# xiph/daala

Measured on AMD Instinct MI355X. Metric: 1080p all-intra transform blocks/s (filter+DCT+PVQ), higher is better.
Workload: dtype int32 (lifting DCT/filters) + f64 (PVQ search)

## Files before the change

### daala_amd/csrc/pvq_refbands.hip

```cpp
#include "../../include/daala_hip.h"
#include <math.h>
#include <stdio.h>
#include <stdlib.h>
#include <string.h>
#include "od_ctx.cuh"
#include "od_pvq_math.cuh"
#include "od_occupancy.cuh"
#include "od_krange.cuh"
#include "od_band_stage.cuh"
#include "gen/od_scan_tables.h"
#define OD_RSQ_TABLE_N 512
#define OD_RSQ_HUGE
#include "pvq_search.cuh"
#include "pvq_row.cuh"
#include "pvq_regs.cuh"
#include "pvq_lane.cuh"

namespace {

constexpr int kMaxJobs = 8;
constexpr int kMaxItems = kMaxJobs*ODHIP_MAX_BANDS;
constexpr int kSlots = ODHIP_PVQ_REF_SLOTS;
constexpr int kUncCap = 1 << 16;
constexpr double kDefaultMargin = 1e-9;
// ... 59 lines not shown
    const int yv = (int16_t)(yw[e >> 1] >> (16*(e & 1)));
    const int qmi = (int16_t)(qw[e >> 1] >> (16*(e & 1)));
    rv[e] = odq_shr_round(odq_mult16_32_q16(yv, ch.z)*qmi, ch.w);
  }
}

__device__ __forceinline__ void lref_piece(const RJob &jb, int band, long blk, int c0, int (&rv)[8]) {
  const long lblk = lref_block(jb, blk);
  const int4 ch = reinterpret_cast<const int4 *>(jb.lchoice)[lblk*jb.lnb + band];
  uint4 y4 = make_uint4(0, 0, 0, 0);
  if (ch.y != 0) y4 = *reinterpret_cast<const uint4 *>(jb.ly + ((long)ch.x*jb.lnblocks + lblk)*jb.llen + c0);
  lref_dequant(ch, y4, *reinterpret_cast<const uint4 *>(jb.lqmi + c0), rv);
}

struct Unc;
struct PUncR {
  int job;
  int band;
  unsigned blk;
  int reserved;
  double rate[ODHIP_PVQ_REF_SLOTS + 1];
};
constexpr int kPUncCap = 1 << 14;

struct RItems : ItemTable<kMaxItems> {
  int perturb;
  double lambda;
  double margin;
  const RJob *jobs;
  unsigned *unc_count;
  Unc *unc;
  unsigned *pcount;
  struct PUncR *plist;
  double tol_scale;
  int fuse;
  int sort_weights;
#ifdef ODHIP_EXPERIMENTS
  int abl;
#endif
};

struct Unc {
  int job;
  int band;
  unsigned blk;
  int theta;
  double corr;
};

__constant__ unsigned char kRScanXY[OD_SCAN_LEN][2];

__device__ __forceinline__ long block_base(const RJob &j, long blk) {
  const int N = 4 << j.bs;
  const long per = (long)j.bw*j.bh;
  const int p = (int)(blk/per);
// ... 61 lines not shown
  const int proj_shift = (odq_ilog(abs(proj)) - 1) - 14;
  const int16_t proj_norm = (int16_t)odq_vshr_round(proj, proj_shift);
  *proj_1 = (int16_t)odq_mult16_16_q15(proj_norm, rcp);
  int os = 14 - proj_shift - 1 + l2r_shift;
  *outshift = os > 30 ? 30 : os;
}


constexpr int kSortBins = 256;
constexpr int kSortChunk = 2048;

__device__ __forceinline__ int od_work_bin(int pulses) {
  if (pulses < 96) return pulses;
  const int b = 96 + ((pulses - 96) >> 3);
  return b < kSortBins ? b : kSortBins - 1;
}

template <class Sink>
__device__ __forceinline__ void refb_enumerate(const RJob &jb, int band, int32_t cg, int32_t gain_offset,
 int32_t theta, int flags, double corr, Sink &sink) {
  const int n = jb.off[band + 1] - jb.off[band];
  const int beta = jb.beta[band];
  if (flags & ODHIP_REFBAND_THETA) {
    int nth = 0;
    const int gain_bound = (cg - gain_offset) >> ODQ_CGAIN_SHIFT;
    const double scale_1 = __ddiv_rn(1., kThetaScale);
    for (int i = gain_bound - 1 > 1 ? gain_bound - 1 : 1; i <= gain_bound + 1; i++) {
      const int32_t qcg = odq_shl32(i, ODQ_CGAIN_SHIFT) + gain_offset;
      const int ts = odq_pvq_compute_max_theta(qcg, beta);
      const double t = __ddiv_rn(((theta*scale_1)*2), kPi)*ts;
      int lower = (int)floor(.5 + t) - 2;
      if (lower < 0) lower = 0;
      int upper = (int)ceil(t);
      if (upper > ts - 1) upper = ts - 1;
      const int gi = i - (gain_bound - 1);
      sink.gain(gi, i, ts, lower);
      for (int j = lower; j <= upper && nth < ODHIP_PVQ_REF_SLOTS - 2; j++) {
        sink.theta(gi, i, j, ts, odq_compute_k_ref(j, n));
        nth++;
      }
    }
  }
  if ((jb.is_keyframe && jb.pli == 0) || corr < .5 || cg < odq_shl32(2, ODQ_CGAIN_SHIFT)) {
    const int gain_bound = cg >> ODQ_CGAIN_SHIFT;
    int c = 0;
    for (int i = gain_bound > 1 ? gain_bound : 1; i <= gain_bound + 1; i++) {
      sink.noref(c++, i, odq_compute_k_noref(odq_shl32(i, ODQ_CGAIN_SHIFT), n, beta));
    }
  }
}

struct KeySink {
  int kt = 0;
  int kn = 0;
  int c = 0;
  unsigned long long mt = 0;
  unsigned long long mn = 0;
  __device__ __forceinline__ void gain(int, int, int, int) {}
// ... 23 lines not shown
    if (fabs(u - rint(u)) < it.margin) {
      flags |= ODHIP_REFBAND_UNCERTAIN;
      if (it.perturb & 1) theta += 1;
      const unsigned slot = atomicAdd(it.unc_count, 1u);
      if (slot < (unsigned)kUncCap) {
        Unc e;
        e.job = job;
        e.band = band;
        e.blk = (unsigned)blk;
        e.theta = theta;
        e.corr = p.corr;
        it.unc[slot] = e;
      }
    }
  }
  odhip_pvq_refband o;
  o.xshift = xshift;
  o.rshift = rshift;
  o.g = p.g;
  o.gr = p.gr;
  o.cg = p.cg;
  o.cgr = p.cgr;
  o.icgr = p.icgr;
  o.gain_offset = p.gain_offset;
  o.m = (int16_t)m;
  o.s = (int8_t)s;
  o.flags = (uint8_t)flags;
  o.theta = theta;
  o.nitems = 0;
  o.ntheta = 0;
  o.corr = p.corr;
  o.dist0 = p.dist0;
  *rec = o;
  if (it.fuse == 2) {
    KeySink ks;
    refb_enumerate(jb, band, o.cg, o.gain_offset, o.theta, flags, o.corr, ks);
    jb.keys[(long)band*jb.nblocks + blk] = (unsigned short)(kSortBins - 1 - od_work_bin(ks.work(it.sort_weights)));
    if (ks.kt > ODHIP_PVQ_MAX_K || ks.kn > ODHIP_PVQ_MAX_K) atomicAdd(jb.krange, 1u);
  }
}

__device__ __forceinline__ uint32_t pack16(int lo, int hi) {
  return (uint32_t)(lo & 0xffff) | (uint32_t)hi << 16;
}

template <int E, class YGet>
__device__ __forceinline__ void store_pulses(int16_t *dst, YGet y) {
  constexpr int SH = E == 15 ? 1 : 0;
  static_assert((E + SH) % 8 == 0, "whole 16-byte pieces");
  uint4 *p = reinterpret_cast<uint4 *>(dst - SH);
  int t[E + SH];
  if (SH) t[0] = 0;
#pragma unroll
  for (int i = 0; i < E; i++) t[i + SH] = y(i);
// ... 191 lines not shown
    for (int i = 0; i < N; i++) {
      int32_t tmp = odq_mult16_16(r16[i], proj_1);
      tmp = outshift >= 0 ? odq_shr_round(tmp, outshift) : odq_shl32(tmp, -outshift);
      v[i] = (int16_t)(x16[i] - tmp);
    }
#pragma unroll
    for (int i = 0; i < N - 1; i++) xr[i] = i < m ? v[i] : v[i + 1];
  }
#ifdef ODHIP_EXPERIMENTS
  const bool abl_nostore = (it.abl & 1) != 0;
  const bool abl_norec = (it.abl & 4) != 0;
#else
  constexpr bool abl_nostore = false;
  constexpr bool abl_norec = false;
#endif
  if (abl_nostore) {
  }
  else if (N == 15) {
    uint4 *xo = reinterpret_cast<uint4 *>(x16o);
    uint4 *ro = reinterpret_cast<uint4 *>(r16o);
    uint4 *xro4 = reinterpret_cast<uint4 *>(xro);
    xo[0] = make_uint4(pack16(0, x16[0]), pack16(x16[1], x16[2]), pack16(x16[3], x16[4]),
     pack16(x16[5], x16[6]));
    xo[1] = make_uint4(pack16(x16[7], x16[8]), pack16(x16[9], x16[10]), pack16(x16[11], x16[12]),
     pack16(x16[13], x16[N - 1]));
    ro[0] = make_uint4(pack16(0, r16[0]), pack16(r16[1], r16[2]), pack16(r16[3], r16[4]),
     pack16(r16[5], r16[6]));
    ro[1] = make_uint4(pack16(r16[7], r16[8]), pack16(r16[9], r16[10]), pack16(r16[11], r16[12]),
     pack16(r16[13], r16[N - 1]));
    xro4[0] = make_uint4(pack16(0, xr[0]), pack16(xr[1], xr[2]), pack16(xr[3], xr[4]),
     pack16(xr[5], xr[6]));
    xro4[1] = make_uint4(pack16(xr[7], xr[8]), pack16(xr[9], xr[10]), pack16(xr[11], xr[12]),
     pack16(xr[13], 0));
  }
  else {
    *reinterpret_cast<uint4 *>(x16o + off) = make_uint4(pack16(x16[0], x16[1]), pack16(x16[2], x16[3]),
     pack16(x16[4], x16[5]), pack16(x16[6], x16[7]));
    *reinterpret_cast<uint4 *>(r16o + off) = make_uint4(pack16(r16[0], r16[1]), pack16(r16[2], r16[3]),
     pack16(r16[4], r16[5]), pack16(r16[6], r16[7]));
    *reinterpret_cast<uint4 *>(xro + off) = make_uint4(pack16(xr[0], xr[1]), pack16(xr[2], xr[3]),
     pack16(xr[4], xr[5]), pack16(xr[6], 0));
  }
  if (!abl_norec) {
    prep_write(it, jb, jb.rec + blk*jb.nb_bands + band, job, band, blk, xshift, rshift, p, r_null, flip, m, s);
  }
}

__global__ __launch_bounds__(kWave) void k_refb_prep_corner(RItems it) {
  const int item = find_item(it, blockIdx.x);
  const int job = __builtin_amdgcn_readfirstlane(it.job[item]);
  const RJob jb = it.jobs[job];
  const long blk = (long)(blockIdx.x - it.wg_start[item])*kWave + threadIdx.x;
  if (blk >= jb.nblocks) return;
  const bool more = jb.nb_bands > 1;
  const int w = jb.w;
  const long base = block_base(jb, blk);
// ... 128 lines not shown
      lref_piece(jb, band, blk, 0, lo);
      lref_piece(jb, band, blk, 8, hi);
#pragma unroll
      for (int i = 0; i < N; i++) rv[i] = i + 1 < 8 ? lo[(i + 1) & 7] : hi[(i + 1) & 7];
    }
    else {
      int pc[8];
      lref_piece(jb, band, blk, off, pc);
#pragma unroll
      for (int i = 0; i < N; i++) rv[i] = pc[i & 7];
    }
  }
  int flip = 0;
  if (jb.is_keyframe && jb.pli != 0) {
    if constexpr (N == 15) flip = cfl_flip15(xv, rv, const_table(jb.qm + off));
    else flip = (jb.rec[blk*jb.nb_bands].flags & ODHIP_REFBAND_FLIP) != 0;
  }
  prep_lane_band<N>(it, jb, job, band, blk, off, xv, rv, flip);
}
#endif

template <int E, int G>
__global__ __launch_bounds__(kWave) void k_refb_prep_row(RItems it) {
  constexpr int n = G*E;
  __shared__ unsigned short s_scan[n];
  const int item = find_item(it, blockIdx.x);
  const int job = it.job[item];
  const RJob &jb = it.jobs[job];
  const int band = it.band[item];
  const int off = jb.off[band];
  const int lane = threadIdx.x;
  for (int j = lane; j < n; j += kWave) s_scan[j] = gRScanPk[off + j];
  __syncthreads();
  const int row = lane/G;
  const int l = lane%G;
  const long nblocks = jb.nblocks;
  const long blk0 = (long)(blockIdx.x - it.wg_start[item])*(kWave/G) + row;
  const bool live = blk0 < nblocks;
  const long blk = live ? blk0 : nblocks - 1;
  const int w = jb.w;
  const int len = jb.len;
  const int nb_bands = jb.nb_bands;
  const int q0 = job_q(jb, band, blk);
  const int beta = jb.beta[band];
  const int is_keyframe = jb.is_keyframe;
  const int cfl_enabled = is_keyframe && jb.pli != 0;
  const long base = block_base(jb, blk);
  const od_coeff *x0 = jb.coef + base;
  const bool lref = jb.ly != nullptr;
  const od_coeff *r0 = lref ? jb.coef + base : jb.ref + base;
  const int16_t *qmp = jb.qm + off + l*E;
  odhip_pvq_refband *rec = jb.rec + blk*nb_bands;
  int16_t *x16o = jb.x16 + blk*len + off;
  int16_t *r16o = jb.r16 + blk*len + off;
  int16_t *xro = jb.xr + blk*len + off;
  const int flip = cfl_enabled ? (rec[0].flags & ODHIP_REFBAND_FLIP) != 0 : 0;
  int xv[E];
  int rv[E];
  int qm[E];
  int sx = 0;
  int sr = 0;
  int nz = 0;
#pragma unroll
  for (int e = 0; e < E; e++) {
    const int pk = s_scan[l*E + e];
    const long p = (long)(pk >> 8)*w + (pk & 255);
    xv[e] = x0[p];
    const int r = lref ? 0 : r0[p];
    rv[e] = flip ? -r : r;
    qm[e] = qmp[e];
  }
// ... 82 lines not shown
    l2r = grp_sum<G>(l2r);
    proj = grp_sum<G>(proj);
    int16_t proj_1;
    int outshift;
    householder_consts(l2r, proj, &proj_1, &outshift);
#pragma unroll
    for (int e = 0; e < E; e++) {
      const int i = l*E + e;
      int32_t tmp = odq_mult16_16(r16[e], proj_1);
      tmp = outshift >= 0 ? odq_shr_round(tmp, outshift) : odq_shl32(tmp, -outshift);
      const int16_t v = (int16_t)(x16[e] - tmp);
      if (live && i != m) xro[i - (i > m)] = v;
    }
  }
  if (live) {
    if constexpr (E == 8) {
      *reinterpret_cast<uint4 *>(x16o + l*E) = make_uint4(pack16(x16[0], x16[1]),
       pack16(x16[2], x16[3]), pack16(x16[4], x16[5]), pack16(x16[6], x16[7]));
      *reinterpret_cast<uint4 *>(r16o + l*E) = make_uint4(pack16(r16[0], r16[1]),
       pack16(r16[2], r16[3]), pack16(r16[4], r16[5]), pack16(r16[6], r16[7]));
    }
    else {
#pragma unroll
      for (int e = 0; e < E; e += 2) {
        *reinterpret_cast<uint32_t *>(x16o + l*E + e) = pack16(x16[e], x16[e + 1]);
        *reinterpret_cast<uint32_t *>(r16o + l*E + e) = pack16(r16[e], r16[e + 1]);
      }
    }
    if (l == 0) prep_write(it, jb, rec + band, job, band, blk, xshift, rshift, p, r_null, flip, m, s);
  }
}


struct ItemPtr {
  int4 *head;
  int4 *tail;
  int4 *res;
  long stride;
};

__device__ __forceinline__ ItemPtr item_ptr(const RJob &jb, int band, long blk) {
  ItemPtr p;
  const long plane = (long)jb.nb_bands*kSlots*jb.nblocks;
  p.head = reinterpret_cast<int4 *>(jb.items) + (long)band*kSlots*jb.nblocks + blk;
// ... 548 lines not shown
  return l == 0 ? 0 : t;
}

template <int G>
__device__ __forceinline__ int grp_total(int v) {
  if constexpr (G == 1) return v;
  else if constexpr (G == 2) return od_grp_add<2>(v);
  else return grp_sum<G>(v);
}

struct RefOutcome {
  int qg;
  int skip;
};

__device__ __forceinline__ RefOutcome refb_decide(const RItems &it, int job, const RJob &jb, int band, long blk,
 const odhip_pvq_refband &r, const RefBest &best, bool writer, int4 *ch) {
  const int cfl_enabled = jb.is_keyframe && jb.pli != 0;
  const int noref = best.noref;
  RefOutcome o;
  o.qg = 0;
  int itheta = jb.is_keyframe ? -1 : 0;
  int max_theta = 0;
  int best_k = 0;
  if (best.close && writer) {
    const unsigned slot = atomicAdd(it.pcount, 1u);
    if (slot < (unsigned)kPUncCap) {
      PUncR *e = it.plist + slot;
      e->job = job;
      e->band = band;
      e->blk = (unsigned)blk;
    }
// ... 20 lines not shown
    if (qg == r.icgr && itheta == 0 && !cfl_enabled) o.skip = 2;
  }
  if (writer) {
    ch[0] = make_int4(best.chosen, qg, noref, itheta);
    ch[1] = make_int4(max_theta, best_k, o.skip, jb.is_keyframe ? (noref ? qg : neg_interleave(qg, r.icgr))
     : (noref ? qg - 1 : neg_interleave(qg + 1, r.icgr + 1)));
  }
  if (o.skip && writer) {
    const int flip = (r.flags & ODHIP_REFBAND_FLIP) != 0;
    ch[2] = make_int4(o.skip == 2 ? (flip ? 4 : 1) : 0, -1, 0, 0);
    ch[3] = make_int4(0, 0, 0, 0);
  }
  return o;
}

template <int E, int G, bool STORE, class YGet>
__device__ __forceinline__ void refb_finish(const RItems &it, int job, const RJob &jb, int band, long blk,
 const odhip_pvq_refband &r, const RefBest &best, int l, bool live, YGet y) {
  constexpr int SH = E == 15 ? 1 : 0;
  static_assert(G == 1 || SH == 0, "only a whole band in one lane starts inside a 16-byte piece");
  const bool writer = live && l == 0;
  int4 *ch = reinterpret_cast<int4 *>(jb.choice + (blk*jb.nb_bands + band)*16);
  const RefOutcome o = refb_decide(it, job, jb, band, blk, r, best, writer, ch);
  if (o.skip) return;
  const int noref = best.noref;
  const int yslot = best.yslot;
  const long at = blk*jb.len + jb.off[band] + l*E;
  int wy[E];
#pragma unroll
  for (int e = 0; e < E; e++) wy[e] = y(e);
  if (STORE && live && yslot >= 0) store_pulses<E>(jb.y + at, [&](int e) -> int { return wy[e]; });
  const int32_t g = odq_gain_expand(odq_shl32(o.qg, ODQ_CGAIN_SHIFT) + (noref ? 0 : r.gain_offset),
   job_q(jb, band, blk), jb.beta[band]);
// ... 9 lines not shown
  gshift = gshift > 0 ? gshift : 0;
  int32_t scale = 0;
  if (yy != 0) {
    int rsqrt_shift;
    const int16_t rsqrt = odq_rsqrt(yy, &rsqrt_shift);
    scale = odq_vshr_round(rsqrt*(int64_t)g, rsqrt_shift + gshift - 16);
  }
  const int qshift = ODQ_QM_INV_SHIFT - gshift;
  if (noref) {
    if (writer) {
      ch[2] = make_int4(2, yslot, scale, qshift);
      ch[3] = make_int4(0, 0, 0, 0);
    }
    return;
  }
  const odhip_pvq_refband *rec = jb.rec + (blk*jb.nb_bands + band);
  const int m = rec->m;
  const int s = rec->s;
  scale = (int32_t)floor(.5 + (scale*(1./32768))*odq_pvq_sin(best.qtheta));
  const int16_t xm = (int16_t)floor(.5 + ((-s*odq_shr_round(g, gshift))*(1./32768))*odq_pvq_cos(best.qtheta));
  uint32_t rw[(E + SH)/2];
  {
    const uint4 *rp = reinterpret_cast<const uint4 *>(jb.r16 + at - SH);
#pragma unroll
    for (int q = 0; q < (E + SH)/8; q++) {
      const uint4 r4 = rp[q];
      rw[4*q] = r4.x;
      rw[4*q + 1] = r4.y;
      rw[4*q + 2] = r4.z;
      rw[4*q + 3] = r4.w;
    }
  }
  const int yprev = grp_from_prev<G>(wy[E - 1], l);
// ... 269 lines not shown
    while (pos > 0) {
      const uint32_t q = col[(pos - 1)*stride];
      if ((q & 0x3ffffu) <= (c & 0x3ffffu)) break;
      if (writer) col[pos*stride] = q;
      pos--;
    }
    if (writer) col[pos*stride] = c;
    n++;
  }
  __device__ __forceinline__ void noref(int c, int, int k) {
    if (writer) col[n*stride] = (uint32_t)c | (uint32_t)(k < 65535 ? k : 65535) << 2;
    n++;
  }
};

__device__ __forceinline__ CandList refb_build_list(const RJob &jb, int band, const odhip_pvq_refband &r,
 uint32_t *col, int stride, bool writer) {
  ListSink sink;
  sink.col = col;
  sink.stride = stride;
  sink.writer = writer;
  CandList cl;
  cl.col = col;
  cl.stride = stride;
  cl.gb1 = ((r.cg - r.gain_offset) >> ODQ_CGAIN_SHIFT) - 1;
  const int gbn = r.cg >> ODQ_CGAIN_SHIFT;
  cl.gbn = gbn > 1 ? gbn : 1;
  struct Split {
    ListSink &s;
    int ntheta = -1;
    __device__ __forceinline__ void gain(int gi, int i, int ts, int lower) { s.gain(gi, i, ts, lower); }
// ... 20 lines not shown
  ThetaCand c;
  c.gi = (int)(w & 3u);
  c.i = cl.gb1 + c.gi;
  c.ts = (int)cl.col[(kSlots + c.gi)*cl.stride];
  c.j = (int)cl.col[(kSlots + 3 + c.gi)*cl.stride] + (int)(w >> 18);
  return c;
}

struct ThetaGate {
  int32_t qcg;
  int32_t qtheta;
  int cosd;
  bool skip;
};

__device__ __forceinline__ ThetaGate refb_theta_gate(const odhip_pvq_refband &r, const ThetaCand &c, int k,
 double lambda) {
  ThetaGate g;
  g.qcg = odq_shl32(c.i, ODQ_CGAIN_SHIFT) + r.gain_offset;
  g.qtheta = odq_pvq_compute_theta(c.j, c.ts);
  g.cosd = odq_pvq_cos(r.theta - g.qtheta);
  g.skip = (refb_dist_gate(g.qcg, r.cg, refb_cos_term(g.cosd)) > r.dist0 + 1.0*lambda && k != 0)
   || k > ODHIP_PVQ_MAX_K;
  return g;
}

struct PreInline {
  ThetaGate g;
  __device__ __forceinline__ void prepare(const odhip_pvq_refband &, const CandList &, double) {}
  __device__ __forceinline__ bool skip(const odhip_pvq_refband &r, const ThetaCand &c, int, int k, double lambda) {
    g = refb_theta_gate(r, c, k, lambda);
    return g.skip;
  }
  __device__ __forceinline__ void values(const odhip_pvq_refband &r, const ThetaCand &, int, int32_t &qcg,
   double &sin_prod) const {
    qcg = g.qcg;
    sin_prod = refb_sin_prod(odq_pvq_sin(r.theta), odq_pvq_sin(g.qtheta));
  }
  __device__ __forceinline__ double cos_term(const odhip_pvq_refband &r, int) const {
    return refb_cos_term(odq_pvq_cos(r.theta - g.qtheta));
  }
};

template <int G, class Store>
__device__ __forceinline__ void refb_prepass(const odhip_pvq_refband &r, const CandList &cl, double lambda, int l,
 Store store) {
  for (int c = l; c < kSlots; c += G) {
    if (c < cl.ntheta) {
      const uint32_t w = cl.col[c*cl.stride];
      store(c, refb_theta_gate(r, theta_cand(cl, w), (int)(w >> 2 & 0xffffu), lambda));
    }
  }
}

template <int WAVES>
__device__ __forceinline__ void refb_prepass_fence(void) {
  if constexpr (WAVES == 1) __syncthreads();
  else {
    __builtin_amdgcn_fence(__ATOMIC_RELEASE, "wavefront");
    __builtin_amdgcn_wave_barrier();
    __builtin_amdgcn_fence(__ATOMIC_ACQUIRE, "wavefront");
  }
}

constexpr int kPreWords = 6;
template <int G, int WAVES>
struct PreLds {
  uint32_t *pre;
  int stride;
  int l;
  double cos = 0;
  __device__ __forceinline__ void prepare(const odhip_pvq_refband &r, const CandList &cl, double lambda) {
    refb_prepass<G>(r, cl, lambda, l, [&](int c, const ThetaGate &g) {
      const double cos_term = refb_cos_term(g.cosd);
      const double sin_prod = refb_sin_prod(odq_pvq_sin(r.theta), odq_pvq_sin(g.qtheta));
      uint32_t *p = pre + c*kPreWords*stride;
      p[0] = (uint32_t)g.qcg;
      p[stride] = g.skip;
      p[2*stride] = (uint32_t)__double2loint(cos_term);
      p[3*stride] = (uint32_t)__double2hiint(cos_term);
      p[4*stride] = (uint32_t)__double2loint(sin_prod);
      p[5*stride] = (uint32_t)__double2hiint(sin_prod);
    });
    refb_prepass_fence<WAVES>();
  }
  __device__ __forceinline__ bool skip(const odhip_pvq_refband &, const ThetaCand &, int idx, int, double) const {
    return pre[(idx*kPreWords + 1)*stride] != 0;
  }
  __device__ __forceinline__ void values(const odhip_pvq_refband &, const ThetaCand &, int idx, int32_t &qcg,
   double &sin_prod) {
    const uint32_t *p = pre + idx*kPreWords*stride;
    qcg = (int32_t)p[0];
    cos = __hiloint2double((int)p[3*stride], (int)p[2*stride]);
    sin_prod = __hiloint2double((int)p[5*stride], (int)p[4*stride]);
  }
  __device__ __forceinline__ double cos_term(const odhip_pvq_refband &, int) const { return cos; }
};

constexpr int kPrePacked = 1;
template <int G, int WAVES>
struct PrePacked {
  static_assert((G == 2 || G == 4) && kSlots <= 32, "the parts of a group's skip mask");
  uint32_t *pre;
  int stride;
  int l;
  uint32_t skips = 0;
  double cos = 0;
  __device__ __forceinline__ void prepare(const odhip_pvq_refband &r, const CandList &cl, double lambda) {
    refb_prepass<G>(r, cl, lambda, l, [&](int c, const ThetaGate &g) {
      skips |= (uint32_t)g.skip << c;
      pre[c*kPrePacked*stride] = ((uint32_t)g.cosd & 0xffffu) | (uint32_t)odq_pvq_sin(g.qtheta) << 16;
    });
    skips = od_grp_or<G>(skips);
    refb_prepass_fence<WAVES>();
  }
  __device__ __forceinline__ bool skip(const odhip_pvq_refband &, const ThetaCand &, int idx, int, double) const {
    return (skips >> idx & 1u) != 0;
  }
  __device__ __forceinline__ void values(const odhip_pvq_refband &r, const ThetaCand &c, int idx, int32_t &qcg,
   double &sin_prod) {
    const uint32_t cs = pre[idx*kPrePacked*stride];
    qcg = odq_shl32(c.i, ODQ_CGAIN_SHIFT) + r.gain_offset;
    cos = refb_cos_term((int16_t)(cs & 0xffffu));
    sin_prod = refb_sin_prod(odq_pvq_sin(r.theta), (int16_t)(cs >> 16));
  }
  __device__ __forceinline__ double cos_term(const odhip_pvq_refband &, int) const { return cos; }
};

template <class D>
__device__ __forceinline__ int lean_k(const D &dec, uint32_t w) {
#ifdef ODHIP_EXPERIMENTS
  if (dec.abl & 8) return 0;
#endif
  (void)dec;
  return (int)(w >> 2 & 0xffffu);
}

template <int NR, class Pre, class V, class D>
__device__ __forceinline__ void refb_loops_lean(const RJob &jb, int band, long blk, const odhip_pvq_refband &r,
 const CandList &cl, double lambda, V &v, D &dec, Pre &pre) {
  const int off = jb.off[band];
  const int n = jb.off[band + 1] - off;
  const int len = jb.len;
  const int32_t cg = r.cg;
  pre.prepare(r, cl, lambda);
  if (cl.ntheta > 0) {
    v.load(jb.xr + blk*len + off, true);
    int prev_k = 0;
    bool has = false;
    double cos_dist = 0;
    double prate = 0;
    int idx = 0;
    while (idx < cl.ntheta) {
      const uint32_t w = cl.col[idx*cl.stride];
// ... 50 lines not shown
template <int NY>
struct LeanDecide {
  double best_cost;
  int chosen;
  bool close;
  int y[NY];
  typename LeanSigns<NY>::type sg;
  double lambda;
  double tol_scale;
  int icgr;
  int is_keyframe;
  int pli;
#ifdef ODHIP_EXPERIMENTS
  int abl = 0;
#endif
  __device__ __forceinline__ void init(const odhip_pvq_refband &r, const RJob &jb, double lam, double tol) {
    best_cost = r.dist0;
    chosen = -1;
    close = false;
    lambda = lam;
    tol_scale = tol;
    icgr = r.icgr;
    is_keyframe = jb.is_keyframe;
    pli = jb.pli;
    sg = 0;
#pragma unroll
    for (int i = 0; i < NY; i++) y[i] = 0;
  }
  template <class V>
  __device__ __forceinline__ void offer(int idx, bool with_ref, int i, int j, double dist, double prate,
   double lts, bool has, const V &v) {
// ... 44 lines not shown
  }
  return b;
}

template <int E, int G>
struct LeanBand {
  int wave;
  int lane;
  int row;
  int l;
  int job;
  int band;
  const RJob *jb;
  bool live;
  long blk;
  odhip_pvq_refband r;
  CandList cl;
  LeanDecide<E> dec;
};

template <int E, int G, int WAVES>
__device__ __forceinline__ bool lean_band(const RItems &it, uint32_t (&s_list_w)[WAVES][kLeanWords*(kWave/G)],
 LeanBand<E, G> &b) {
  constexpr int C = kWave/G;
  b.wave = __builtin_amdgcn_readfirstlane(threadIdx.x/kWave);
  const int unit = blockIdx.x*WAVES + b.wave;
  if (unit >= it.wg_start[it.nitems]) return false;
  const int item = find_item(it, unit);
  b.job = it.job[item];
  b.jb = &it.jobs[b.job];
  b.band = it.band[item];
  b.lane = threadIdx.x%kWave;
  b.row = b.lane/G;
  b.l = b.lane%G;
  const RJob &jb = *b.jb;
  const long nblocks = jb.nblocks;
  const long pos = (long)(unit - it.wg_start[item])*C + b.row;
  b.live = pos < nblocks;
  if (G == 1 && !b.live) return false;
  b.blk = jb.ids[(long)b.band*nblocks + (b.live ? pos : nblocks - 1)];
  b.r = jb.rec[b.blk*jb.nb_bands + b.band];
  b.cl = refb_build_list(jb, b.band, b.r, s_list_w[b.wave] + b.row, C, b.l == 0);
  b.dec.init(b.r, jb, it.lambda, it.tol_scale);
#ifdef ODHIP_EXPERIMENTS
  b.dec.abl = it.abl;
#endif
  return true;
}

template <int N>
__global__ __launch_bounds__(kSearchThreads) OD_SEARCH_OCC_ATTR void k_refb_lean_lane(RItems it) {
  __shared__ uint32_t s_list_w[kSearchWaves][kLeanWords*kWave];
  OD_SEARCH_VGPR_FLOOR();
  od_rsqrt_init(threadIdx.x);
  LeanBand<N, 1> b;
  if (!lean_band<N, 1, kSearchWaves>(it, s_list_w, b)) return;
// ... 294 lines not shown
    d.lqmi = l.d_qm_inv;
    d.lsplit = (long)l.nplanes*d.bw*d.bh;
    d.lnblocks = d.lsplit;
    d.llen = ln*ln < OD_SCAN_LEN ? ln*ln : OD_SCAN_LEN;
    d.lnb = OD_NBANDS[l.bs];
  }
  return ODHIP_SUCCESS;
}

struct RefState {
  long theta_listed = 0;
  JobTables<RJob, kMaxJobs> tabs;
  Counters<3> counters;
  DeviceBuf<Unc> unc;
  DeviceBuf<PUncR> plist;
  PinnedCount unc_posted;
  PinnedCount priced;
  BlockSort<kSortBins, kSortChunk, RJob, kMaxItems> sort;
  SideStreams streams;
  ProfEvents prof;
  double margin = kDefaultMargin;
  int perturb = 0;
  double tol_scale = 1.;
  bool lean = false;
  unsigned *unc_count() const { return counters.d.p; }
  unsigned *pcount() const { return counters.d.p + 1; }
};

int ref_state(RefState **out) {
  ODHIP_CTX_OR_RETURN(ctx);
// ... 42 lines not shown
  return w;
}

void items_begin(RItems &it, const RefState &st, double lambda) {
  memset(&it, 0, sizeof(it));
  it.lambda = lambda;
  it.margin = st.margin;
  it.perturb = st.perturb;
  it.jobs = st.tabs.cur;
  it.unc_count = st.unc_count();
  it.unc = st.unc.p;
  it.pcount = st.pcount();
  it.plist = st.plist.p;
  it.tol_scale = st.tol_scale;
  it.sort_weights = sort_weights();
#ifdef ODHIP_EXPERIMENTS
  static const int abl = [] {
    const char *e = getenv("ODHIP_REFB_ABL");
    return e ? atoi(e) : 0;
  }();
  it.abl = abl;
#endif
}

enum RefStage {
  kStageRecords = 0,
  kStageLanePriced = 1,
  kStageDecided = 2
};

// ... 118 lines not shown
    }
#endif
  }
  if (st.streams.join(s, side) != ODHIP_SUCCESS) return ODHIP_EFAULT;
  return ODHIP_SUCCESS;
}

int ref_bands(const odhip_pvq_refjob *jobs, int njobs, double pvq_norm_lambda, odhip_stream stream, RefStage stage) {
  hipStream_t s = (hipStream_t)stream;
  REF_STATE_OR_RETURN(st);
  RJob host[kMaxJobs];
  int rc = stage_jobs(st, jobs, njobs, kJobBands, host, s);
  if (rc) return rc;
  ODHIP_TRY(hipMemsetAsync(st.unc_count(), 0, (stage != kStageRecords ? 2 : 1)*sizeof(unsigned), s));
  st.lean = stage == kStageDecided;
  RItems it;
  items_begin(it, st, pvq_norm_lambda);
  items_add_size(it, host, njobs, 0, kWave);
  if (!it.nitems) return ODHIP_SUCCESS;
  launch_prep(st, host, njobs, pvq_norm_lambda, stage, s);
  if (stage != kStageDecided) k_refb_cands<<<it.wg_start[it.nitems], kWave, 0, s>>>(it);
  rc = sort_blocks(st, host, njobs, s);
  if (rc) return rc;
  rc = launch_searches(st, host, njobs, pvq_norm_lambda, stage, s);
  if (rc) return rc;
  if (stage == kStageDecided) {
    rc = st.unc_posted.post(st.unc_count(), s);
    if (!rc) rc = st.priced.post(st.pcount(), s);
    if (rc) return rc;
  }
  return odhip_check_launch();
}

void rerun_listed(const RefState &st, const Unc *d_list, unsigned n, double lambda, hipStream_t s) {
  k_refb_cands_list<<<(n + kWave - 1)/kWave, kWave, 0, s>>>(st.tabs.cur, d_list, (int)n);
  k_refb_search_list<<<n, kWave, (size_t)2*128*kWave*sizeof(unsigned short), s>>>(st.tabs.cur, d_list, (int)n,
   lambda);
}

void decide_listed(RefState &st, const Unc *d_list, unsigned n, double lambda, hipStream_t s) {
  RItems it;
  items_begin(it, st, lambda);
  const unsigned grid = (n + kWave - 1)/kWave;
  for (const int size : kBandSizes) {
    for_band_size(size, [&](auto N) {
      k_refb_choose_unc_list<decltype(N)::value><<<grid, kWave, 0, s>>>(it, d_list, (int)n);
    });
  }
  (void)st.priced.post(st.pcount(), s);
}

enum RefSelect {
// ... 114 lines not shown
  for (int i = 0; i < count; i++) {
    const int32_t theta = (int32_t)floor(.5 + (32768*2./M_PI)*acos(list[i].corr));
    if (theta != list[i].theta) {
      list[nfix] = list[i];
      list[nfix].theta = theta;
      nfix++;
    }
  }
  if (nfix == 0) return 0;
  RJob host[kMaxJobs];
  int rc = stage_jobs(st, jobs, njobs, kJobBands, host, s);
  if (rc) return rc;
  if (!listed_jobs_valid(list.data(), nfix, njobs)) return ODHIP_EINVAL;
  DeviceBuf<Unc> d_list;
  if (upload_list(d_list, list.data(), nfix, &s)) return ODHIP_EFAULT;
  rerun_listed(st, d_list.p, nfix, pvq_norm_lambda, s);
  if (st.lean) decide_listed(st, d_list.p, nfix, pvq_norm_lambda, s);
  rc = odhip_check_launch();
  const hipError_t e = hipStreamSynchronize(s);
  if (rc) return rc;
  if (e != hipSuccess) return ODHIP_EFAULT;
  return (int)nfix;
}

int odhip_pvq_ref_resolve_finish(const odhip_pvq_refjob *jobs, int njobs, double pvq_norm_lambda,
 odhip_stream stream) {
  REF_STATE_OR_RETURN(st);
  const int posted = st.unc_posted.wait();
  if (posted <= 0) return posted;
  return odhip_pvq_ref_resolve(jobs, njobs, pvq_norm_lambda, stream);
// ... 41 lines not shown
    catch (const std::bad_alloc &) {
      return ODHIP_EFAULT;
    }
    for (int i = 0; i < count; i++) {
      ul[i].job = list[i].job;
      ul[i].band = list[i].band;
      ul[i].blk = list[i].blk;
      ul[i].theta = -1;
      ul[i].corr = 0;
    }
    DeviceBuf<Unc> d_ul;
    if (upload_list(d_ul, ul.data(), count)) return ODHIP_EFAULT;
    RJob host0[kMaxJobs];
    rc = stage_jobs(st, jobs, njobs, kJobBands, host0, s);
    if (rc) return rc;
    rerun_listed(st, d_ul.p, count, pvq_norm_lambda, s);
    rc = odhip_check_launch();
    if (hipStreamSynchronize(s) != hipSuccess) rc = ODHIP_EFAULT;
    if (!rc) rc = stage_jobs(st, jobs, njobs, kJobChoice, host, s);
    if (rc) return rc;
  }
  for (PUncR &e : list) {
    const RJob &jb = host[e.job];
    const int n = jb.off[e.band + 1] - jb.off[e.band];
    const long B = jb.nblocks;
    odhip_pvq_refband rec;
    ODHIP_TRY(hipMemcpy(&rec, jb.rec + (long)e.blk*jb.nb_bands + e.band, sizeof(rec), hipMemcpyDeviceToHost));
    const int4 *head = reinterpret_cast<const int4 *>(jb.items) + (long)e.band*kSlots*B + e.blk;
    const int4 *tail = head + (long)jb.nb_bands*kSlots*B;
    for (int c = 0; c <= kSlots; c++) e.rate[c] = 0;
// ... 46 lines not shown
```

Before: 1.317 billion.

## Write compact lean per-band records and skip unused x/xr stores in fused mode

In the fused (lean) decide path, the prep kernels now write a compact 32-byte LeanRec per band into a separate buffer instead of the full odhip_pvq_refband record. They also skip storing x16 when no no-ref candidates exist and xr when no Householder reflection was applied. The lean decide kernels read the compact record and unpack the derived values. The uncertain-list rerun paths gain a new prep_list kernel that rebuilds full records for listed bands. This cuts global write and read traffic in the common path, at the cost of an extra buffer, more code paths, and an added kernel launch on the resolve paths.

```diff
diff --git a/daala_amd/csrc/pvq_refbands.hip b/daala_amd/csrc/pvq_refbands.hip
--- a/daala_amd/csrc/pvq_refbands.hip
+++ b/daala_amd/csrc/pvq_refbands.hip
@@ -97,6 +97,42 @@
 }
 
 struct Unc;
+struct LeanRec {
+  int32_t cg;
+  int32_t cgr;
+  int32_t theta;
+  uint32_t msf;
+  double corr;
+  double dist0;
+};
+static_assert(sizeof(LeanRec) == 32, "two records to a 64-byte line");
+
+struct LeanVals {
+  int32_t cg;
+  int32_t gain_offset;
+  int32_t icgr;
+  int32_t theta;
+  int flags;
+  double corr;
+  double dist0;
+};
+
+__device__ __forceinline__ uint32_t lean_msf(int m, int s, int flags) {
+  return (uint32_t)(uint16_t)m | (uint32_t)(uint8_t)s << 16 | (uint32_t)flags << 24;
+}
+
+__device__ __forceinline__ LeanVals lean_vals(const LeanRec &m) {
+  LeanVals r;
+  r.cg = m.cg;
+  r.icgr = odq_shr_round(m.cgr, ODQ_CGAIN_SHIFT);
+  r.gain_offset = m.cgr - odq_shl32(r.icgr, ODQ_CGAIN_SHIFT);
+  r.theta = m.theta;
+  r.flags = (int)(m.msf >> 24);
+  r.corr = m.corr;
+  r.dist0 = m.dist0;
+  return r;
+}
+
 struct PUncR {
   int job;
   int band;
@@ -121,7 +157,18 @@
 #ifdef ODHIP_EXPERIMENTS
   int abl;
 #endif
+  LeanRec *lean;
+  long lean_at[kMaxJobs];
 };
+
+__device__ __forceinline__ LeanRec *lean_rec(const RItems &it, int job, const RJob &jb, long blk, int band) {
+  return it.lean + (it.lean_at[job] + blk*jb.nb_bands + band);
+}
+
+__device__ __forceinline__ int block_flip(const RItems &it, int job, const RJob &jb, long blk, bool lean) {
+  const int flags = lean ? (int)(lean_rec(it, job, jb, blk, 0)->msf >> 24) : jb.rec[blk*jb.nb_bands].flags;
+  return (flags & ODHIP_REFBAND_FLIP) != 0;
+}
 
 struct Unc {
   int job;
@@ -213,6 +260,10 @@
   if (pulses < 96) return pulses;
   const int b = 96 + ((pulses - 96) >> 3);
   return b < kSortBins ? b : kSortBins - 1;
+}
+
+__device__ __forceinline__ bool refb_has_noref(const RJob &jb, int32_t cg, double corr) {
+  return (jb.is_keyframe && jb.pli == 0) || corr < .5 || cg < odq_shl32(2, ODQ_CGAIN_SHIFT);
 }
 
 template <class Sink>
@@ -240,7 +291,7 @@
       }
     }
   }
-  if ((jb.is_keyframe && jb.pli == 0) || corr < .5 || cg < odq_shl32(2, ODQ_CGAIN_SHIFT)) {
+  if (refb_has_noref(jb, cg, corr)) {
     const int gain_bound = cg >> ODQ_CGAIN_SHIFT;
     int c = 0;
     for (int i = gain_bound > 1 ? gain_bound : 1; i <= gain_bound + 1; i++) {
@@ -294,6 +345,21 @@
       }
     }
   }
+  if (it.fuse == 2) {
+    LeanRec o;
+    o.cg = p.cg;
+    o.cgr = p.cgr;
+    o.theta = theta;
+    o.msf = lean_msf(m, s, flags);
+    o.corr = p.corr;
+    o.dist0 = p.dist0;
+    *lean_rec(it, job, jb, blk, band) = o;
+    KeySink ks;
+    refb_enumerate(jb, band, p.cg, p.gain_offset, theta, flags, p.corr, ks);
+    jb.keys[(long)band*jb.nblocks + blk] = (unsigned short)(kSortBins - 1 - od_work_bin(ks.work(it.sort_weights)));
+    if (ks.kt > ODHIP_PVQ_MAX_K || ks.kn > ODHIP_PVQ_MAX_K) atomicAdd(jb.krange, 1u);
+    return;
+  }
   odhip_pvq_refband o;
   o.xshift = xshift;
   o.rshift = rshift;
@@ -312,12 +378,6 @@
   o.corr = p.corr;
   o.dist0 = p.dist0;
   *rec = o;
-  if (it.fuse == 2) {
-    KeySink ks;
-    refb_enumerate(jb, band, o.cg, o.gain_offset, o.theta, flags, o.corr, ks);
-    jb.keys[(long)band*jb.nblocks + blk] = (unsigned short)(kSortBins - 1 - od_work_bin(ks.work(it.sort_weights)));
-    if (ks.kt > ODHIP_PVQ_MAX_K || ks.kn > ODHIP_PVQ_MAX_K) atomicAdd(jb.krange, 1u);
-  }
 }
 
 __device__ __forceinline__ uint32_t pack16(int lo, int hi) {
@@ -539,32 +599,42 @@
   constexpr bool abl_nostore = false;
   constexpr bool abl_norec = false;
 #endif
+  const bool keep_x = it.fuse != 2 || refb_has_noref(jb, p.cg, p.corr);
+  const bool keep_xr = it.fuse != 2 || p.ran;
   if (abl_nostore) {
   }
   else if (N == 15) {
     uint4 *xo = reinterpret_cast<uint4 *>(x16o);
     uint4 *ro = reinterpret_cast<uint4 *>(r16o);
     uint4 *xro4 = reinterpret_cast<uint4 *>(xro);
-    xo[0] = make_uint4(pack16(0, x16[0]), pack16(x16[1], x16[2]), pack16(x16[3], x16[4]),
-     pack16(x16[5], x16[6]));
-    xo[1] = make_uint4(pack16(x16[7], x16[8]), pack16(x16[9], x16[10]), pack16(x16[11], x16[12]),
-     pack16(x16[13], x16[N - 1]));
+    if (keep_x) {
+      xo[0] = make_uint4(pack16(0, x16[0]), pack16(x16[1], x16[2]), pack16(x16[3], x16[4]),
+       pack16(x16[5], x16[6]));
+      xo[1] = make_uint4(pack16(x16[7], x16[8]), pack16(x16[9], x16[10]), pack16(x16[11], x16[12]),
+       pack16(x16[13], x16[N - 1]));
+    }
     ro[0] = make_uint4(pack16(0, r16[0]), pack16(r16[1], r16[2]), pack16(r16[3], r16[4]),
      pack16(r16[5], r16[6]));
     ro[1] = make_uint4(pack16(r16[7], r16[8]), pack16(r16[9], r16[10]), pack16(r16[11], r16[12]),
      pack16(r16[13], r16[N - 1]));
-    xro4[0] = make_uint4(pack16(0, xr[0]), pack16(xr[1], xr[2]), pack16(xr[3], xr[4]),
-     pack16(xr[5], xr[6]));
-    xro4[1] = make_uint4(pack16(xr[7], xr[8]), pack16(xr[9], xr[10]), pack16(xr[11], xr[12]),
-     pack16(xr[13], 0));
+    if (keep_xr) {
+      xro4[0] = make_uint4(pack16(0, xr[0]), pack16(xr[1], xr[2]), pack16(xr[3], xr[4]),
+       pack16(xr[5], xr[6]));
+      xro4[1] = make_uint4(pack16(xr[7], xr[8]), pack16(xr[9], xr[10]), pack16(xr[11], xr[12]),
+       pack16(xr[13], 0));
+    }
   }
   else {
-    *reinterpret_cast<uint4 *>(x16o + off) = make_uint4(pack16(x16[0], x16[1]), pack16(x16[2], x16[3]),
-     pack16(x16[4], x16[5]), pack16(x16[6], x16[7]));
+    if (keep_x) {
+      *reinterpret_cast<uint4 *>(x16o + off) = make_uint4(pack16(x16[0], x16[1]), pack16(x16[2], x16[3]),
+       pack16(x16[4], x16[5]), pack16(x16[6], x16[7]));
+    }
     *reinterpret_cast<uint4 *>(r16o + off) = make_uint4(pack16(r16[0], r16[1]), pack16(r16[2], r16[3]),
      pack16(r16[4], r16[5]), pack16(r16[6], r16[7]));
-    *reinterpret_cast<uint4 *>(xro + off) = make_uint4(pack16(xr[0], xr[1]), pack16(xr[2], xr[3]),
-     pack16(xr[4], xr[5]), pack16(xr[6], 0));
+    if (keep_xr) {
+      *reinterpret_cast<uint4 *>(xro + off) = make_uint4(pack16(xr[0], xr[1]), pack16(xr[2], xr[3]),
+       pack16(xr[4], xr[5]), pack16(xr[6], 0));
+    }
   }
   if (!abl_norec) {
     prep_write(it, jb, jb.rec + blk*jb.nb_bands + band, job, band, blk, xshift, rshift, p, r_null, flip, m, s);
@@ -723,28 +793,19 @@
   int flip = 0;
   if (jb.is_keyframe && jb.pli != 0) {
     if constexpr (N == 15) flip = cfl_flip15(xv, rv, const_table(jb.qm + off));
-    else flip = (jb.rec[blk*jb.nb_bands].flags & ODHIP_REFBAND_FLIP) != 0;
+    else flip = block_flip(it, job, jb, blk, it.fuse == 2);
   }
   prep_lane_band<N>(it, jb, job, band, blk, off, xv, rv, flip);
 }
 #endif
 
 template <int E, int G>
-__global__ __launch_bounds__(kWave) void k_refb_prep_row(RItems it) {
+__device__ __forceinline__ void prep_row_band(const RItems &it, int job, const RJob &jb, int band, long blk0,
+ bool lean_flip, const unsigned short *s_scan) {
   constexpr int n = G*E;
-  __shared__ unsigned short s_scan[n];
-  const int item = find_item(it, blockIdx.x);
-  const int job = it.job[item];
-  const RJob &jb = it.jobs[job];
-  const int band = it.band[item];
   const int off = jb.off[band];
-  const int lane = threadIdx.x;
-  for (int j = lane; j < n; j += kWave) s_scan[j] = gRScanPk[off + j];
-  __syncthreads();
-  const int row = lane/G;
-  const int l = lane%G;
+  const int l = threadIdx.x%G;
   const long nblocks = jb.nblocks;
-  const long blk0 = (long)(blockIdx.x - it.wg_start[item])*(kWave/G) + row;
   const bool live = blk0 < nblocks;
   const long blk = live ? blk0 : nblocks - 1;
   const int w = jb.w;
@@ -763,7 +824,7 @@
   int16_t *x16o = jb.x16 + blk*len + off;
   int16_t *r16o = jb.r16 + blk*len + off;
   int16_t *xro = jb.xr + blk*len + off;
-  const int flip = cfl_enabled ? (rec[0].flags & ODHIP_REFBAND_FLIP) != 0 : 0;
+  const int flip = cfl_enabled ? block_flip(it, job, jb, blk, lean_flip) : 0;
   int xv[E];
   int rv[E];
   int qm[E];
@@ -876,20 +937,106 @@
     }
   }
   if (live) {
+    const bool keep_x = it.fuse != 2 || refb_has_noref(jb, p.cg, p.corr);
     if constexpr (E == 8) {
-      *reinterpret_cast<uint4 *>(x16o + l*E) = make_uint4(pack16(x16[0], x16[1]),
-       pack16(x16[2], x16[3]), pack16(x16[4], x16[5]), pack16(x16[6], x16[7]));
+      if (keep_x) {
+        *reinterpret_cast<uint4 *>(x16o + l*E) = make_uint4(pack16(x16[0], x16[1]),
+         pack16(x16[2], x16[3]), pack16(x16[4], x16[5]), pack16(x16[6], x16[7]));
+      }
       *reinterpret_cast<uint4 *>(r16o + l*E) = make_uint4(pack16(r16[0], r16[1]),
        pack16(r16[2], r16[3]), pack16(r16[4], r16[5]), pack16(r16[6], r16[7]));
     }
     else {
 #pragma unroll
       for (int e = 0; e < E; e += 2) {
-        *reinterpret_cast<uint32_t *>(x16o + l*E + e) = pack16(x16[e], x16[e + 1]);
+        if (keep_x) *reinterpret_cast<uint32_t *>(x16o + l*E + e) = pack16(x16[e], x16[e + 1]);
         *reinterpret_cast<uint32_t *>(r16o + l*E + e) = pack16(r16[e], r16[e + 1]);
       }
     }
     if (l == 0) prep_write(it, jb, rec + band, job, band, blk, xshift, rshift, p, r_null, flip, m, s);
+  }
+}
+
+template <int E, int G>
+__global__ __launch_bounds__(kWave) void k_refb_prep_row(RItems it) {
+  constexpr int n = G*E;
+  __shared__ unsigned short s_scan[n];
+  const int item = find_item(it, blockIdx.x);
+  const int job = it.job[item];
+  const RJob &jb = it.jobs[job];
+  const int band = it.band[item];
+  const int off = jb.off[band];
+  const int lane = threadIdx.x;
+  for (int j = lane; j < n; j += kWave) s_scan[j] = gRScanPk[off + j];
+  __syncthreads();
+  const long blk0 = (long)(blockIdx.x - it.wg_start[item])*(kWave/G) + lane/G;
+  prep_row_band<E, G>(it, job, jb, band, blk0, it.fuse == 2, s_scan);
+}
+
+template <int N>
+__device__ __forceinline__ void prep_lane_listed(const RItems &it, int job, const RJob &jb, int band, long blk) {
+  const int off = jb.off[band];
+  const long base = block_base(jb, blk);
+  const bool lref = jb.ly != nullptr;
+  int xv[N];
+  int rv[N];
+#pragma unroll
+  for (int i = 0; i < N; i++) {
+    const long p = base + coef_pos(jb, off + i);
+    xv[i] = jb.coef[p];
+    rv[i] = lref ? 0 : jb.ref[p];
+  }
+  if (lref) {
+    if constexpr (N == 15) {
+      int lo[8];
+      int hi[8];
+      lref_piece(jb, band, blk, 0, lo);
+      lref_piece(jb, band, blk, 8, hi);
+#pragma unroll
+      for (int i = 0; i < N; i++) rv[i] = i + 1 < 8 ? lo[(i + 1) & 7] : hi[(i + 1) & 7];
+    }
+    else {
+      int pc[8];
+      lref_piece(jb, band, blk, off, pc);
+#pragma unroll
+      for (int i = 0; i < N; i++) rv[i] = pc[i & 7];
+    }
+  }
+  int flip = 0;
+  if (jb.is_keyframe && jb.pli != 0) {
+    if constexpr (N == 15) flip = cfl_flip15(xv, rv, const_table(jb.qm + off));
+    else flip = block_flip(it, job, jb, blk, true);
+  }
+  prep_lane_band<N>(it, jb, job, band, blk, off, xv, rv, flip);
+}
+
+__global__ __launch_bounds__(kWave) void k_refb_prep_list(RItems it, const Unc *list, int count) {
+  __shared__ unsigned short s_scan[128];
+  if ((int)blockIdx.x >= count) return;
+  const Unc e = list[blockIdx.x];
+  const int job = e.job;
+  const RJob &jb = it.jobs[job];
+  const int band = e.band;
+  const long blk = e.blk;
+  const int off = jb.off[band];
+  const int n = jb.off[band + 1] - off;
+  const int lane = threadIdx.x;
+  if (n >= 32) {
+    for (int j = lane; j < n; j += kWave) s_scan[j] = gRScanPk[off + j];
+    __syncthreads();
+    if (n == 32) prep_row_band<8, 4>(it, job, jb, band, lane < 4 ? blk : jb.nblocks, true, s_scan);
+    else prep_row_band<8, 16>(it, job, jb, band, lane < 16 ? blk : jb.nblocks, true, s_scan);
+  }
+  else if (lane == 0) {
+    if (n == 15) prep_lane_listed<15>(it, job, jb, band, blk);
+    else prep_lane_listed<8>(it, job, jb, band, blk);
+  }
+  if (lane == 0) {
+    LeanRec *lr = lean_rec(it, job, jb, blk, band);
+    odhip_pvq_refband *rec = jb.rec + blk*jb.nb_bands + band;
+    if (e.theta >= 0) lr->theta = e.theta;
+    rec->theta = lr->theta;
+    rec->flags = (uint8_t)(lr->msf >> 24);
   }
 }
 
@@ -1468,8 +1615,9 @@
   int skip;
 };
 
+template <class R>
 __device__ __forceinline__ RefOutcome refb_decide(const RItems &it, int job, const RJob &jb, int band, long blk,
- const odhip_pvq_refband &r, const RefBest &best, bool writer, int4 *ch) {
+ const R &r, const RefBest &best, bool writer, int4 *ch) {
   const int cfl_enabled = jb.is_keyframe && jb.pli != 0;
   const int noref = best.noref;
   RefOutcome o;
@@ -1520,9 +1668,23 @@
   return o;
 }
 
-template <int E, int G, bool STORE, class YGet>
+__device__ __forceinline__ void band_pivot(const RItems &, int, const RJob &jb, int band, long blk,
+ const odhip_pvq_refband &, int &m, int &s) {
+  const odhip_pvq_refband *rec = jb.rec + (blk*jb.nb_bands + band);
+  m = rec->m;
+  s = rec->s;
+}
+
+__device__ __forceinline__ void band_pivot(const RItems &it, int job, const RJob &jb, int band, long blk,
+ const LeanVals &, int &m, int &s) {
+  const uint32_t w = lean_rec(it, job, jb, blk, band)->msf;
+  m = (int)(w & 0xffffu);
+  s = (int8_t)(w >> 16);
+}
+
+template <int E, int G, bool STORE, class R, class YGet>
 __device__ __forceinline__ void refb_finish(const RItems &it, int job, const RJob &jb, int band, long blk,
- const odhip_pvq_refband &r, const RefBest &best, int l, bool live, YGet y) {
+ const R &r, const RefBest &best, int l, bool live, YGet y) {
   constexpr int SH = E == 15 ? 1 : 0;
   static_assert(G == 1 || SH == 0, "only a whole band in one lane starts inside a 16-byte piece");
   const bool writer = live && l == 0;
@@ -1562,9 +1724,9 @@
     }
     return;
   }
-  const odhip_pvq_refband *rec = jb.rec + (blk*jb.nb_bands + band);
-  const int m = rec->m;
-  const int s = rec->s;
+  int m;
+  int s;
+  band_pivot(it, job, jb, band, blk, r, m, s);
   scale = (int32_t)floor(.5 + (scale*(1./32768))*odq_pvq_sin(best.qtheta));
   const int16_t xm = (int16_t)floor(.5 + ((-s*odq_shr_round(g, gshift))*(1./32768))*odq_pvq_cos(best.qtheta));
   uint32_t rw[(E + SH)/2];
@@ -1864,7 +2026,7 @@
   }
 };
 
-__device__ __forceinline__ CandList refb_build_list(const RJob &jb, int band, const odhip_pvq_refband &r,
+__device__ __forceinline__ CandList refb_build_list(const RJob &jb, int band, const LeanVals &r,
  uint32_t *col, int stride, bool writer) {
   ListSink sink;
   sink.col = col;
@@ -1915,7 +2077,7 @@
   bool skip;
 };
 
-__device__ __forceinline__ ThetaGate refb_theta_gate(const odhip_pvq_refband &r, const ThetaCand &c, int k,
+__device__ __forceinline__ ThetaGate refb_theta_gate(const LeanVals &r, const ThetaCand &c, int k,
  double lambda) {
   ThetaGate g;
   g.qcg = odq_shl32(c.i, ODQ_CGAIN_SHIFT) + r.gain_offset;
@@ -1928,23 +2090,23 @@
 
 struct PreInline {
   ThetaGate g;
-  __device__ __forceinline__ void prepare(const odhip_pvq_refband &, const CandList &, double) {}
-  __device__ __forceinline__ bool skip(const odhip_pvq_refband &r, const ThetaCand &c, int, int k, double lambda) {
+  __device__ __forceinline__ void prepare(const LeanVals &, const CandList &, double) {}
+  __device__ __forceinline__ bool skip(const LeanVals &r, const ThetaCand &c, int, int k, double lambda) {
     g = refb_theta_gate(r, c, k, lambda);
     return g.skip;
   }
-  __device__ __forceinline__ void values(const odhip_pvq_refband &r, const ThetaCand &, int, int32_t &qcg,
+  __device__ __forceinline__ void values(const LeanVals &r, const ThetaCand &, int, int32_t &qcg,
    double &sin_prod) const {
     qcg = g.qcg;
     sin_prod = refb_sin_prod(odq_pvq_sin(r.theta), odq_pvq_sin(g.qtheta));
   }
-  __device__ __forceinline__ double cos_term(const odhip_pvq_refband &r, int) const {
+  __device__ __forceinline__ double cos_term(const LeanVals &r, int) const {
     return refb_cos_term(odq_pvq_cos(r.theta - g.qtheta));
   }
 };
 
 template <int G, class Store>
-__device__ __forceinline__ void refb_prepass(const odhip_pvq_refband &r, const CandList &cl, double lambda, int l,
+__device__ __forceinline__ void refb_prepass(const LeanVals &r, const CandList &cl, double lambda, int l,
  Store store) {
   for (int c = l; c < kSlots; c += G) {
     if (c < cl.ntheta) {
@@ -1971,7 +2133,7 @@
   int stride;
   int l;
   double cos = 0;
-  __device__ __forceinline__ void prepare(const odhip_pvq_refband &r, const CandList &cl, double lambda) {
+  __device__ __forceinline__ void prepare(const LeanVals &r, const CandList &cl, double lambda) {
     refb_prepass<G>(r, cl, lambda, l, [&](int c, const ThetaGate &g) {
       const double cos_term = refb_cos_term(g.cosd);
       const double sin_prod = refb_sin_prod(odq_pvq_sin(r.theta), odq_pvq_sin(g.qtheta));
@@ -1985,17 +2147,17 @@
     });
     refb_prepass_fence<WAVES>();
   }
-  __device__ __forceinline__ bool skip(const odhip_pvq_refband &, const ThetaCand &, int idx, int, double) const {
+  __device__ __forceinline__ bool skip(const LeanVals &, const ThetaCand &, int idx, int, double) const {
     return pre[(idx*kPreWords + 1)*stride] != 0;
   }
-  __device__ __forceinline__ void values(const odhip_pvq_refband &, const ThetaCand &, int idx, int32_t &qcg,
+  __device__ __forceinline__ void values(const LeanVals &, const ThetaCand &, int idx, int32_t &qcg,
    double &sin_prod) {
     const uint32_t *p = pre + idx*kPreWords*stride;
     qcg = (int32_t)p[0];
     cos = __hiloint2double((int)p[3*stride], (int)p[2*stride]);
     sin_prod = __hiloint2double((int)p[5*stride], (int)p[4*stride]);
   }
-  __device__ __forceinline__ double cos_term(const odhip_pvq_refband &, int) const { return cos; }
+  __device__ __forceinline__ double cos_term(const LeanVals &, int) const { return cos; }
 };
 
 constexpr int kPrePacked = 1;
@@ -2007,7 +2169,7 @@
   int l;
   uint32_t skips = 0;
   double cos = 0;
-  __device__ __forceinline__ void prepare(const odhip_pvq_refband &r, const CandList &cl, double lambda) {
+  __device__ __forceinline__ void prepare(const LeanVals &r, const CandList &cl, double lambda) {
     refb_prepass<G>(r, cl, lambda, l, [&](int c, const ThetaGate &g) {
       skips |= (uint32_t)g.skip << c;
       pre[c*kPrePacked*stride] = ((uint32_t)g.cosd & 0xffffu) | (uint32_t)odq_pvq_sin(g.qtheta) << 16;
@@ -2015,17 +2177,17 @@
     skips = od_grp_or<G>(skips);
     refb_prepass_fence<WAVES>();
   }
-  __device__ __forceinline__ bool skip(const odhip_pvq_refband &, const ThetaCand &, int idx, int, double) const {
+  __device__ __forceinline__ bool skip(const LeanVals &, const ThetaCand &, int idx, int, double) const {
     return (skips >> idx & 1u) != 0;
   }
-  __device__ __forceinline__ void values(const odhip_pvq_refband &r, const ThetaCand &c, int idx, int32_t &qcg,
+  __device__ __forceinline__ void values(const LeanVals &r, const ThetaCand &c, int idx, int32_t &qcg,
    double &sin_prod) {
     const uint32_t cs = pre[idx*kPrePacked*stride];
     qcg = odq_shl32(c.i, ODQ_CGAIN_SHIFT) + r.gain_offset;
     cos = refb_cos_term((int16_t)(cs & 0xffffu));
     sin_prod = refb_sin_prod(odq_pvq_sin(r.theta), (int16_t)(cs >> 16));
   }
-  __device__ __forceinline__ double cos_term(const odhip_pvq_refband &, int) const { return cos; }
+  __device__ __forceinline__ double cos_term(const LeanVals &, int) const { return cos; }
 };
 
 template <class D>
@@ -2038,7 +2200,7 @@
 }
 
 template <int NR, class Pre, class V, class D>
-__device__ __forceinline__ void refb_loops_lean(const RJob &jb, int band, long blk, const odhip_pvq_refband &r,
+__device__ __forceinline__ void refb_loops_lean(const RJob &jb, int band, long blk, const LeanVals &r,
  const CandList &cl, double lambda, V &v, D &dec, Pre &pre) {
   const int off = jb.off[band];
   const int n = jb.off[band + 1] - off;
@@ -2119,7 +2281,7 @@
 #ifdef ODHIP_EXPERIMENTS
   int abl = 0;
 #endif
-  __device__ __forceinline__ void init(const odhip_pvq_refband &r, const RJob &jb, double lam, double tol) {
+  __device__ __forceinline__ void init(const LeanVals &r, const RJob &jb, double lam, double tol) {
     best_cost = r.dist0;
     chosen = -1;
     close = false;
@@ -2194,7 +2356,7 @@
   const RJob *jb;
   bool live;
   long blk;
-  odhip_pvq_refband r;
+  LeanVals r;
   CandList cl;
   LeanDecide<E> dec;
 };
@@ -2219,7 +2381,7 @@
   b.live = pos < nblocks;
   if (G == 1 && !b.live) return false;
   b.blk = jb.ids[(long)b.band*nblocks + (b.live ? pos : nblocks - 1)];
-  b.r = jb.rec[b.blk*jb.nb_bands + b.band];
+  b.r = lean_vals(*lean_rec(it, b.job, jb, b.blk, b.band));
   b.cl = refb_build_list(jb, b.band, b.r, s_list_w[b.wave] + b.row, C, b.l == 0);
   b.dec.init(b.r, jb, it.lambda, it.tol_scale);
 #ifdef ODHIP_EXPERIMENTS
@@ -2544,6 +2706,8 @@
   Counters<3> counters;
   DeviceBuf<Unc> unc;
   DeviceBuf<PUncR> plist;
+  DeviceBuf<LeanRec> lean_rec;
+  long lean_at[kMaxJobs] = {};
   PinnedCount unc_posted;
   PinnedCount priced;
   BlockSort<kSortBins, kSortChunk, RJob, kMaxItems> sort;
@@ -2616,6 +2780,8 @@
   it.plist = st.plist.p;
   it.tol_scale = st.tol_scale;
   it.sort_weights = sort_weights();
+  it.lean = st.lean_rec.p;
+  for (int j = 0; j < kMaxJobs; j++) it.lean_at[j] = st.lean_at[j];
 #ifdef ODHIP_EXPERIMENTS
   static const int abl = [] {
     const char *e = getenv("ODHIP_REFB_ABL");
@@ -2764,6 +2930,15 @@
   if (rc) return rc;
   ODHIP_TRY(hipMemsetAsync(st.unc_count(), 0, (stage != kStageRecords ? 2 : 1)*sizeof(unsigned), s));
   st.lean = stage == kStageDecided;
+  if (st.lean) {
+    size_t recs = 0;
+    for (int j = 0; j < njobs; j++) {
+      st.lean_at[j] = (long)recs;
+      recs += (size_t)host[j].nblocks*host[j].nb_bands;
+    }
+    rc = st.lean_rec.grow(recs, s);
+    if (rc) return rc;
+  }
   RItems it;
   items_begin(it, st, pvq_norm_lambda);
   items_add_size(it, host, njobs, 0, kWave);
@@ -2786,6 +2961,14 @@
   k_refb_cands_list<<<(n + kWave - 1)/kWave, kWave, 0, s>>>(st.tabs.cur, d_list, (int)n);
   k_refb_search_list<<<n, kWave, (size_t)2*128*kWave*sizeof(unsigned short), s>>>(st.tabs.cur, d_list, (int)n,
    lambda);
+}
+
+void prep_listed(const RefState &st, const Unc *d_list, unsigned n, double lambda, hipStream_t s) {
+  RItems it;
+  items_begin(it, st, lambda);
+  it.fuse = kStageRecords;
+  it.margin = 0;
+  k_refb_prep_list<<<n, kWave, 0, s>>>(it, d_list, (int)n);
 }
 
 void decide_listed(RefState &st, const Unc *d_list, unsigned n, double lambda, hipStream_t s) {
@@ -2930,6 +3113,7 @@
   if (!listed_jobs_valid(list.data(), nfix, njobs)) return ODHIP_EINVAL;
   DeviceBuf<Unc> d_list;
   if (upload_list(d_list, list.data(), nfix, &s)) return ODHIP_EFAULT;
+  if (st.lean) prep_listed(st, d_list.p, nfix, pvq_norm_lambda, s);
   rerun_listed(st, d_list.p, nfix, pvq_norm_lambda, s);
   if (st.lean) decide_listed(st, d_list.p, nfix, pvq_norm_lambda, s);
   rc = odhip_check_launch();
@@ -3001,6 +3185,7 @@
     RJob host0[kMaxJobs];
     rc = stage_jobs(st, jobs, njobs, kJobBands, host0, s);
     if (rc) return rc;
+    prep_listed(st, d_ul.p, count, pvq_norm_lambda, s);
     rerun_listed(st, d_ul.p, count, pvq_norm_lambda, s);
     rc = odhip_check_launch();
     if (hipStreamSynchronize(s) != hipSuccess) rc = ODHIP_EFAULT;
```

Result: faster. 1.333 billion (median of 6 runs) (+1.2%).
